# patrickltobing/shallow-wavenet

Measured on AMD Instinct MI355X. Metric: decoded samples/sec (22.05 kHz Laplacian AR decode, whole job), higher is better.
Workload: dtype f32

## Files before the change

shallow_wavenet_amd/csrc/swn_decode_bl6w.hip:

```cpp
#include <type_traits>
#include "swn_decode_bl6_common.hpp"
#include "swn_decode_internal.hpp"

#ifndef SWN_RES_SLICE
#define SWN_RES_SLICE 0
#endif
#ifndef SWN_ROTATE
#define SWN_ROTATE 1
#endif
#ifndef SWN_HANDOFF
#define SWN_HANDOFF 0
#endif
#ifndef SWN_OLDER2_MERGED
#define SWN_OLDER2_MERGED 1
#endif
#ifndef SWN_EARLY_ROWS
#define SWN_EARLY_ROWS 1
#endif

namespace {

using namespace swn_bl6;

constexpr int NG = 256;
constexpr int S = 128;
constexpr int O1 = 128;

template <int LPC_, bool EXT_>
struct Tw {
    static constexpr int LPC = LPC_;
    static constexpr bool EXT = EXT_;
    using Ext = Tw<LPC_, true>;
    static constexpr bool NEWFORM = !EXT_ && LPC_ == 0;
    static constexpr int NO = 2 + LPC_;
    static constexpr int WN = cmax(1, LPC_) + 1;
    static constexpr int ring_len(int l) { return pow2ceil((1 << l) + 1); }
    static constexpr int ring_off(int l) { int o = 0; for (int i = 0; i < l; ++i) o += ring_len(i) * H; return o; }
    static constexpr int PF = L * 2 * H;
    static constexpr int NZC = 64, NZB = 4;
    static constexpr int o_ring = 0;
    static constexpr int o_hcat = o_ring + ring_off(L);
    static constexpr int o_gp = o_hcat + L * H;
    static constexpr int o_bx = o_gp + 2 * PF;
    static constexpr int o_bd = o_bx + L * 2 * H;
    static constexpr int o_old = o_bd + L * 2 * H;
    static constexpr int o_wup = o_old + 2 * L * 2 * H;
    static constexpr int o_skip = o_wup + 256;
    static constexpr int o_p2 = o_skip + S;
    static constexpr int o_tnz = o_p2 + 4 * NO;
    static constexpr int o_cz = o_tnz + r4(NZB * NZC);
    static constexpr int o_w2 = o_cz + 5 * H;
    static constexpr int o_bias = o_w2 + NO * S + r4(NO);
    static constexpr int o_w1 = o_bias + S + O1;
    static constexpr int o_wl = o_w1 + 8 * O1 * 16;
    static constexpr int o_h0w = o_wl + 8 * NG * 4;
    static constexpr int o_ho = o_h0w + 3 * H;
    static constexpr int HO = 4, NHO = 128;
    static constexpr int o_end = o_ho + (NEWFORM && (SWN_HANDOFF & 1) && SWN_ROTATE ? NHO * HO : 0);
    static constexpr size_t lds_bytes = (size_t)o_end * sizeof(float);
    static constexpr int sess_old = ring_off(L);
    static constexpr int sess_win = sess_old + 2 * L * 2 * H;
    static constexpr int sess_floats = sess_win + r4(WN);
};

__device__ __forceinline__ float sum_quads(float v) {
    v += dpp_f<0x124>(v);
    v += dpp_f<0x128>(v);
    float w = v;
    asm("s_nop 1\n\tv_permlane16_swap_b32 %0, %1" : "+v"(v), "+v"(w));
    v += w;
    w = v;
    asm("s_nop 1\n\tv_permlane32_swap_b32 %0, %1" : "+v"(v), "+v"(w));
    return v + w;
}
__device__ __forceinline__ float quad_sum_by_parity(float own, float other) {
    float s = own + dpp_f<0xB1>(other);
    s += dpp_f<0x4E>(s);
    return s;
}
struct NoWork { __device__ __forceinline__ void operator()() const {} };
template <class T, int LAYER, int NQ = 2, class BEHIND = NoWork>
__device__ __forceinline__ void layer_a(float* lds, const float (&w)[2][16], const int q, const float wj, const int pb, const int po,
                                        const int ta, const float* xr, BEHIND&& behind = NoWork{}) {
    constexpr bool ROT = !std::is_same<typename std::decay<BEHIND>::type, NoWork>::value;
    const int o = ta >> 2, p = ta & 3, pr = p & 1;
    const float e_old = lds[T::o_old + po + LAYER * 2 * H + pr * H + o];
    const float g_gp = lds[T::o_gp + pb + LAYER * 2 * H + pr * H + o], g_bx = lds[T::o_bx + LAYER * 2 * H + pr * H + o];
    const float e_hp = xr[o];
    static_assert(NQ >= 0 && NQ <= 4, "early quads");
    float4 xq[4];
    if constexpr (ROT) {
#pragma unroll
        for (int m = 0; m < NQ; ++m) xq[m] = *reinterpret_cast<const float4*>(xr + 16 * p + 4 * m);
        __builtin_amdgcn_sched_barrier(0);
        behind();
        __builtin_amdgcn_sched_barrier(0);
    }
    const float e_gx = fmaf(wj, g_gp, g_bx);
    float az = 0.f, ac = 0.f;
#pragma unroll
    for (int m = 0; m < 4; ++m) {
        float4 x;
        if (ROT && m < NQ) x = xq[m];
        else x = *reinterpret_cast<const float4*>(xr + 16 * p + 4 * m);
        az = fmaf(w[0][4 * m], x.x, az); ac = fmaf(w[1][4 * m], x.x, ac);
        az = fmaf(w[0][4 * m + 1], x.y, az); ac = fmaf(w[1][4 * m + 1], x.y, ac);
        az = fmaf(w[0][4 * m + 2], x.z, az); ac = fmaf(w[1][4 * m + 2], x.z, ac);
        az = fmaf(w[0][4 * m + 3], x.w, az); ac = fmaf(w[1][4 * m + 3], x.w, ac);
    }
    const float sq = quad_sum_by_parity(pr ? ac : az, pr ? az : ac);
    __builtin_amdgcn_sched_barrier(0);
    if (p < 2) {
        const float sa = sq + e_old;
        const float v = e_gx * sa;
        const float e = exp_c(p == 0 ? -v : -2.f * fminf(fabsf(v), 64.f));
        const float r = rcp_c(1.f + e);
        const float res = p == 0 ? r : copysignf((1.f - e) * r, v);
        const float c = dpp_f<0xF5>(res);
        if (p == 0) {
            const float hn = (1.f - res) * c + res * e_hp;
            if (LAYER + 1 < L) {
                constexpr int R2 = T::ring_len(LAYER + 1 < L ? LAYER + 1 : LAYER);
                lds[T::o_ring + T::ring_off(LAYER + 1 < L ? LAYER + 1 : LAYER) + (q & (R2 - 1)) * H + o] = hn;
            }
            lds[T::o_hcat + LAYER * H + o] = hn;
        }
    }
    __builtin_amdgcn_sched_barrier(0);
}

template <class T, int LAYER, int MB = 4>
__device__ __forceinline__ void older_sum(const float* lds, const float (&w)[2][16], const int qn, const int tb, float& az, float& ac) {
    constexpr int dil = 1 << LAYER;
    constexpr int R = T::ring_len(LAYER);
    const int p = tb & 3;
    const float* ring = lds + T::o_ring + T::ring_off(LAYER);
    az = 0.f; ac = 0.f;
#pragma unroll
    for (int m = 0; m < 4; ++m) {
        const float4 x = *reinterpret_cast<const float4*>(ring + ((qn - dil) & (R - 1)) * H + 16 * p + 4 * m);
        float4 w0, w1;
        if (LAYER < L - 1) {
            w0 = make_float4(w[0][4 * m], w[0][4 * m + 1], w[0][4 * m + 2], w[0][4 * m + 3]);
            w1 = make_float4(w[1][4 * m], w[1][4 * m + 1], w[1][4 * m + 2], w[1][4 * m + 3]);
        } else {
            w0 = *reinterpret_cast<const float4*>(lds + T::o_wl + (m * NG + tb) * 4);
            w1 = *reinterpret_cast<const float4*>(lds + T::o_wl + ((4 + m) * NG + tb) * 4);
        }
        az = fmaf(w0.x, x.x, az); ac = fmaf(w1.x, x.x, ac);
        az = fmaf(w0.y, x.y, az); ac = fmaf(w1.y, x.y, ac);
        az = fmaf(w0.z, x.z, az); ac = fmaf(w1.z, x.z, ac);
        az = fmaf(w0.w, x.w, az); ac = fmaf(w1.w, x.w, ac);
        if (MB < 4 && m % MB == MB - 1) __builtin_amdgcn_sched_barrier(0);
    }
    az = sum4(az); ac = sum4(ac);
}
template <class T, int LAYER>
__device__ __forceinline__ void older_store(float* lds, const int qn, const int tb, const float az, const float ac) {
    const int o = tb >> 2, p = tb & 3, pr = p & 1;
    lds[T::o_old + (qn & 1) * (L * 2 * H) + LAYER * 2 * H + pr * H + o] = (p == 0 ? az : ac) + lds[T::o_bd + LAYER * 2 * H + pr * H + o];
}
template <class T, int LAYER, int MB = 4>
__device__ __forceinline__ void older_b(float* lds, const float (&w)[2][16], const int qn, const int tb) {
    float az, ac;
    older_sum<T, LAYER, MB>(lds, w, qn, tb, az, ac);
    if ((tb & 3) < 2) older_store<T, LAYER>(lds, qn, tb, az, ac);
}
template <class T>
__device__ __forceinline__ void older_last_rows(const float* lds, const int qn, const int tb, float4 (&x)[2], float4 (&w)[2][2]) {
    constexpr int LAYER = L - 1, dil = 1 << LAYER, R = T::ring_len(LAYER);
    const float* row = lds + T::o_ring + T::ring_off(LAYER) + ((qn - dil) & (R - 1)) * H + 16 * (tb & 3);
#pragma unroll
    for (int m = 0; m < 2; ++m) {
        x[m] = *reinterpret_cast<const float4*>(row + 4 * m);
        w[m][0] = *reinterpret_cast<const float4*>(lds + T::o_wl + (m * NG + tb) * 4);
        w[m][1] = *reinterpret_cast<const float4*>(lds + T::o_wl + ((4 + m) * NG + tb) * 4);
    }
}
template <class T>
__device__ __forceinline__ void older_last_x(float* lds, const float4 (&xe)[2], const float4 (&we)[2][2], const int qn, const int tb) {
    constexpr int LAYER = L - 1, dil = 1 << LAYER, R = T::ring_len(LAYER);
    const float* row = lds + T::o_ring + T::ring_off(LAYER) + ((qn - dil) & (R - 1)) * H + 16 * (tb & 3);
    float az = 0.f, ac = 0.f;
#pragma unroll
    for (int m = 0; m < 4; ++m) {
        float4 x, w0, w1;
        if (m < 2) { x = xe[m]; w0 = we[m][0]; w1 = we[m][1]; }
        else {
            x = *reinterpret_cast<const float4*>(row + 4 * m);
            w0 = *reinterpret_cast<const float4*>(lds + T::o_wl + (m * NG + tb) * 4);
            w1 = *reinterpret_cast<const float4*>(lds + T::o_wl + ((4 + m) * NG + tb) * 4);
        }
        az = fmaf(w0.x, x.x, az); ac = fmaf(w1.x, x.x, ac);
        az = fmaf(w0.y, x.y, az); ac = fmaf(w1.y, x.y, ac);
        az = fmaf(w0.z, x.z, az); ac = fmaf(w1.z, x.z, ac);
        az = fmaf(w0.w, x.w, az); ac = fmaf(w1.w, x.w, ac);
        if (m == 1) __builtin_amdgcn_sched_barrier(0);
    }
    az = sum4(az); ac = sum4(ac);
    if ((tb & 3) < 2) older_store<T, LAYER>(lds, qn, tb, az, ac);
}
template <int... LS> struct Layers {};
template <class T, int NW, int... LS>
__device__ __forceinline__ void older_bn(Layers<LS...>, float* lds, const float (&w)[NW][2][16], const int qn, const int tb) {
    static_assert(((LS < NW) && ...), "register-resident halves only");
    float az[sizeof...(LS)], ac[sizeof...(LS)];
    int k = 0;
    ((older_sum<T, LS>(lds, w[LS], qn, tb, az[k], ac[k]), ++k), ...);
    if ((tb & 3) < 2) {
        k = 0;
        ((older_store<T, LS>(lds, qn, tb, az[k], ac[k]), ++k), ...);
    }
}

template <class T, int LAYER>
__device__ __forceinline__ void older_rows(const float* lds, const int qn, const int tb, float4 (&x)[4]) {
    constexpr int dil = 1 << LAYER;
    constexpr int R = T::ring_len(LAYER);
    const float* row = lds + T::o_ring + T::ring_off(LAYER) + ((qn - dil) & (R - 1)) * H + 16 * (tb & 3);
#pragma unroll
    for (int m = 0; m < 4; ++m) x[m] = *reinterpret_cast<const float4*>(row + 4 * m);
}
__device__ __forceinline__ void older_sum_x(const float (&w)[2][16], const float4 (&x)[4], float& az, float& ac) {
    az = 0.f; ac = 0.f;
#pragma unroll
    for (int m = 0; m < 4; ++m) {
        az = fmaf(w[0][4 * m], x[m].x, az); ac = fmaf(w[1][4 * m], x[m].x, ac);
        az = fmaf(w[0][4 * m + 1], x[m].y, az); ac = fmaf(w[1][4 * m + 1], x[m].y, ac);
        az = fmaf(w[0][4 * m + 2], x[m].z, az); ac = fmaf(w[1][4 * m + 2], x[m].z, ac);
        az = fmaf(w[0][4 * m + 3], x[m].w, az); ac = fmaf(w[1][4 * m + 3], x[m].w, ac);
    }
    az = sum4(az); ac = sum4(ac);
}
template <class T, int... LS>
__device__ __forceinline__ void older_rows_n(Layers<LS...>, const float* lds, const int qn, const int tb, float4 (&x)[sizeof...(LS)][4]) {
    int k = 0;
    ((older_rows<T, LS>(lds, qn, tb, x[k]), ++k), ...);
}
template <class T, int NW, int... LS>
__device__ __forceinline__ void older_bn_x(Layers<LS...>, float* lds, const float (&w)[NW][2][16], const float4 (&x)[sizeof...(LS)][4],
                                           const int qn, const int tb) {
    static_assert(((LS < NW) && ...), "register-resident halves only");
    float az[sizeof...(LS)], ac[sizeof...(LS)];
    int k = 0;
    ((older_sum_x(w[LS], x[k], az[k], ac[k]), ++k), ...);
    if ((tb & 3) < 2) {
        k = 0;
        ((older_store<T, LS>(lds, qn, tb, az[k], ac[k]), ++k), ...);
    }
}

template <int LAYER>
__device__ __forceinline__ void skip_issue_b(__amdgpu_buffer_rsrc_t wsk2, float4 (&wsl)[8], const int tb, const unsigned step0) {
    const int r = tb >> 2, hp = tb & 3;
#pragma unroll
    for (int ps = 0; ps < 2; ++ps)
#pragma unroll
        for (int mm = 0; mm < 4; ++mm)
            wsl[ps * 4 + mm] = buf_ld4(wsk2, (unsigned)((r + 64 * ps) * 4 + hp) * 16u, (unsigned)((LAYER * 4 + mm) * S) * 64u + step0);
}
template <class T, int LAYER, bool REQ = true>
__device__ __forceinline__ void skip_roll_b(const float* lds, __amdgpu_buffer_rsrc_t wsk2, const float4 (&wcur)[8], float4 (&wnext)[8],
                                            float (&sacc)[2], const int tb, const unsigned step0) {
    static_assert(LAYER >= 1 && LAYER < L, "slice LAYER - 1 in flight, slice LAYER to request");
    const int r = tb >> 2, hp = tb & 3;
    float4 xs[4];
#pragma unroll
    for (int mm = 0; mm < 4; ++mm) xs[mm] = *reinterpret_cast<const float4*>(lds + T::o_hcat + (LAYER - 1) * H + 16 * mm + 4 * hp);
#pragma unroll
    for (int mm = 0; mm < 4; ++mm) {
#pragma unroll
        for (int ps = 0; ps < 2; ++ps) {
            const float4 x = xs[mm], w = wcur[ps * 4 + mm];
            sacc[ps] = fmaf(w.x, x.x, sacc[ps]); sacc[ps] = fmaf(w.y, x.y, sacc[ps]);
            sacc[ps] = fmaf(w.z, x.z, sacc[ps]); sacc[ps] = fmaf(w.w, x.w, sacc[ps]);
        }
        __builtin_amdgcn_sched_barrier(0);
#pragma unroll
        for (int ps = 0; ps < 2; ++ps)
            if (REQ) wnext[ps * 4 + mm] = buf_ld4(wsk2, (unsigned)((r + 64 * ps) * 4 + hp) * 16u, (unsigned)((LAYER * 4 + mm) * S) * 64u + step0);
        __builtin_amdgcn_sched_barrier(0);
    }
    asm volatile("" : "+v"(sacc[0]), "+v"(sacc[1]));
}
template <class T>
__device__ __forceinline__ void skip_last_b(float* lds, const float4 (&wsl)[8], const float (&sacc)[2], const int tb) {
    const int r = tb >> 2, hp = tb & 3;
    float part[2][4];
#pragma unroll
    for (int mm = 0; mm < 4; ++mm) {
        const float4 x = *reinterpret_cast<const float4*>(lds + T::o_hcat + (L - 1) * H + 16 * mm + 4 * hp);
#pragma unroll
        for (int ps = 0; ps < 2; ++ps) {
            const float4 w = wsl[ps * 4 + mm];
            part[ps][mm] = fmaf(w.w, x.w, fmaf(w.z, x.z, fmaf(w.y, x.y, w.x * x.x)));
        }
    }
    float s[2];
#pragma unroll
    for (int ps = 0; ps < 2; ++ps) s[ps] = sacc[ps] + ((part[ps][0] + part[ps][1]) + (part[ps][2] + part[ps][3]));
    const float t0 = s[0] + dpp_f<0xB1>(s[0]), t1 = s[1] + dpp_f<0xB1>(s[1]);
    const float v = (hp < 2 ? t0 : t1) + dpp_f<0x4E>(hp < 2 ? t1 : t0);
    if ((hp & 1) == 0) lds[T::o_skip + r + 32 * hp] = fmaxf(v, 0.f);
}

template <bool MOVE2> using OlderMergedT = typename std::conditional<MOVE2, Layers<2, 3, 4>, Layers<3, 4>>::type;
template <bool MOVE2> using OlderOut1T = typename std::conditional<MOVE2, Layers<0, 1>, Layers<0, 1, 2>>::type;
template <int E> struct Out1Split;
template <> struct Out1Split<2> { using Early = Layers<0, 1>; using Late = Layers<>; };
template <> struct Out1Split<1> { using Early = Layers<0>; using Late = Layers<1>; };
template <> struct Out1Split<0> { using Early = Layers<>; using Late = Layers<0, 1>; };

template <class T, bool GA, bool STREAM, bool POOL = false>
__device__ __forceinline__ void decode_body(const Bl6Args& a, float* lds) {
    constexpr bool EXT = T::EXT;
    static_assert(!STREAM || EXT, "streamed chunks run the extended mode");
    constexpr bool grpA = GA;
    const int tid = threadIdx.x, b = POOL ? 0 : blockIdx.x;
    __builtin_assume(GA ? tid < NG : tid >= NG);
    const int tg = tid & (NG - 1);
    const float* __restrict__ P = a.P;
    const int U = a.U;
    const int s0 = STREAM ? a.step0 : 0;
    const bool resume = STREAM && a.resume;
    const int fb0 = STREAM ? s0 / U : 0;

    for (int e = tid; e < T::o_end; e += NT) lds[e] = 0.f;
    __syncthreads();
    for (int e = tid; e < L * 2 * H; e += NT) {
        lds[T::o_bx + e] = P[a.y.bx + e];
        const float bd = P[a.y.bd + e];
        lds[T::o_bd + e] = bd;
        lds[T::o_old + e] = bd;
    }
    for (int e = tid; e < U; e += NT) lds[T::o_wup + e] = P[a.y.wup + e];
    for (int e = tid; e < H; e += NT) lds[T::o_cz + e] = P[a.y.cb + e];
    for (int e = tid; e < S; e += NT) lds[T::o_bias + e] = P[a.y.bsk + e];
    for (int e = tid; e < O1; e += NT) lds[T::o_bias + S + e] = P[a.y.b1 + e];
    for (int e = tid; e < 2 * H; e += NT) { lds[T::o_cz + H + e] = P[a.y.cv + e]; lds[T::o_cz + 3 * H + e] = P[a.y.cc + e]; }
    for (int e = tid; e < T::NO * S; e += NT) lds[T::o_w2 + e] = P[a.y.w2 + (size_t)(e / S) * r4(S) + (e % S)];
    for (int e = tid; e < T::NO; e += NT) lds[T::o_w2 + T::NO * S + e] = P[a.y.b2 + e];
    for (int e = tid; e < 8 * O1 * 16; e += NT) lds[T::o_w1 + e] = P[a.y.w12 + e];
    const __amdgpu_buffer_rsrc_t condr =
        make_rsrc(a.cond + (size_t)b * a.Tf * a.N, (unsigned)((size_t)a.Tf * a.N * sizeof(float)));
    auto load_frame = [&](int fr) {
        float* dst = lds + T::o_gp + (fr & 1) * T::PF;
#pragma unroll
        for (int it = 0; it < (T::PF / 4 + NT - 1) / NT; ++it) {
            const int e4 = it * NT + tid;
            if (e4 < T::PF / 4)
                *reinterpret_cast<float4*>(dst + 4 * e4) =
                    buf_ld4(condr, (unsigned)tid * 16u, (unsigned)(fr * a.N * 4 + it * NT * 16));
        }
    };
    for (int fr = fb0; fr < fb0 + 2 && fr < a.Tf; ++fr) load_frame(fr);
    constexpr int NWR = grpA ? L : L - 1;
    float wreg[NWR][2][16];
    {
        const int o = tg >> 2, p = tg & 3, k = grpA ? 1 : 0;
#pragma unroll
        for (int l = 0; l < L; ++l)
#pragma unroll
            for (int r = 0; r < 2; ++r) {
                const float4* src = reinterpret_cast<const float4*>(P + a.y.wd + (((size_t)l * 2 * H + o + r * H) * 2 + k) * H + 16 * p);
#pragma unroll
                for (int v = 0; v < 4; ++v) {
                    const float4 t = src[v];
                    if (l == L - 1 && !grpA) {
                        *reinterpret_cast<float4*>(lds + T::o_wl + ((r * 4 + v) * NG + tg) * 4) = t;
                    } else {
                        float (&wr)[16] = wreg[l < NWR ? l : 0][r];
                        wr[4 * v] = t.x; wr[4 * v + 1] = t.y; wr[4 * v + 2] = t.z; wr[4 * v + 3] = t.w;
                    }
                }
            }
    }
    __syncthreads();
    const float* sess_b = STREAM ? a.sess + (size_t)b * T::sess_floats : nullptr;
    int tcp = tid;
    asm volatile("" : "+v"(tcp));
    if (resume) {
        for (int e = tcp; e < T::ring_off(L); e += NT) lds[T::o_ring + e] = sess_b[e];
        for (int e = tcp; e < 2 * L * 2 * H; e += NT) lds[T::o_old + e] = sess_b[T::sess_old + e];
        __syncthreads();
    }

    int fb = fb0, tb0 = fb0 * U;
    const int n_pro = RF;
    auto cond_taps = [&](int q, float& wj, int& pb) {
        const int t0 = q - RF;
        const int tlo = t0 < 0 ? 0 : t0;
        if (tlo >= tb0 + U) {
            fb += 1; tb0 += U;
            if (fb + 1 < a.Tf) load_frame(fb + 1);
        }
        int rel = tlo - tb0;
        int fsel = fb;
        if (rel >= U) { rel -= U; fsel = fb + 1; }
        rel = rel < U ? rel : U - 1;
        wj = lds[T::o_wup + rel];
        pb = (fsel & 1) * T::PF;
    };

    auto input_seed = [&](int q) {
        if (tid < H) {
            const int o = tid;
            float acc = c_b;
#pragma unroll
            for (int k = 0; k < 2; ++k) {
                const int r = q - (1 - k);
                if (r >= 0) acc += fmaf(k ? c_v1 : c_v0, 0.f, k ? c_c1 : c_c0);
            }
            lds[T::o_ring + (q & 1) * H + o] = ssign(acc);
        }
    };
    float win[T::WN];
#pragma unroll
    for (int k = 0; k < T::WN; ++k) win[k] = 0.f;
    if (EXT && a.seed) win[T::WN - 1] = reinterpret_cast<const float*>(a.seed)[b];
    if (resume) {
#pragma unroll
        for (int k = 0; k < T::WN; ++k) win[k] = sess_b[T::sess_win + k];
    }
    const int wv = __builtin_amdgcn_readfirstlane(tg >> 6);
    float kcb = 0.f, kv0 = 0.f, kv1 = 0.f, kc0 = 0.f, kc1 = 0.f;
    if (grpA) { const int o = tg & (H - 1); kcb = c_b; kv0 = c_v0; kv1 = c_v1; kc0 = c_c0; kc1 = c_c1; }
    auto h0_row = [&](int qn) -> int {
        return wv == 0 ? T::o_ring + (qn & 1) * H : T::o_h0w + (wv - 1) * H;
    };
    auto input_gen = [&](int row) {
        if constexpr (grpA) {
            float acc = kcb;
            acc += fmaf(kv0, win[T::WN - 2], kc0);
            acc += fmaf(kv1, win[T::WN - 1], kc1);
            lds[row + (tg & (H - 1))] = ssign(acc);
            lds_fence_compiler();
        }
    };
#ifdef SWN_DIAG_NOSIDE
    constexpr bool NOSIDE = T::NEWFORM;
#else
    constexpr bool NOSIDE = false;
#endif
#ifdef SWN_DIAG_NOSTREAM
    constexpr bool NOSTREAM = T::NEWFORM;
#else
    constexpr bool NOSTREAM = false;
#endif
    constexpr bool HOFF = T::NEWFORM && (SWN_HANDOFF & 7) && SWN_ROTATE;
    constexpr bool HO_ST = HOFF && (SWN_HANDOFF & 1), HO_RF = HOFF && (SWN_HANDOFF & 2), HO_NZ = HOFF && (SWN_HANDOFF & 4);
    constexpr bool MOVE2 = T::NEWFORM && SWN_OLDER2_MERGED;
    using OlderMerged = OlderMergedT<MOVE2>;
    using OlderOut1 = OlderOut1T<MOVE2>;
    constexpr int NOUT1 = MOVE2 ? 2 : 3;
    constexpr int NEARLY = MOVE2 ? SWN_EARLY_ROWS : NOUT1;
    static_assert(NEARLY >= 0 && NEARLY <= NOUT1, "early rows");
    constexpr bool NZG = HO_NZ ? !grpA : grpA;
    const int tn = HO_NZ ? tg : tid;
    float e_next = 0.f;
    auto noise_load = [&](int c) {
        const int step = c * T::NZC + tn - 64;
        if (step < a.n_steps) e_next = a.noise[(size_t)b * a.n_steps + step];
    };
    auto noise_chunk = [&](int c) {
        if (NZG && tn >= 64 && tn < 128) {
            const int k = tn - 64, step = c * T::NZC + k;
            if (step < a.n_steps) {
                const float e = EXT ? swn_noise_laplace_at(a.nz, b, step, s0 + step, 0, a.n_steps, 1) : e_next;
                const float sg = (e > 0.f) ? 1.f : ((e < 0.f) ? -1.f : 0.f);
                lds[T::o_tnz + (c & (T::NZB - 1)) * T::NZC + k] = sg * log1pf(-2.f * fabsf(e));
            }
            if (!EXT) noise_load(c + 1);
        }
    };
    if (!EXT && NZG && tn >= 64 && tn < 128) noise_load(0);
    noise_chunk(0);
    noise_chunk(1);

    const __amdgpu_buffer_rsrc_t wsk2 = make_rsrc(P + a.y.wsk2, (unsigned)(L * S * 64 * sizeof(float)));
    constexpr bool NEWFORM = T::NEWFORM;
    constexpr int RES = (grpA || !NEWFORM) ? -1 : SWN_RES_SLICE;
    static_assert(RES == -1 || RES == 0 || RES == L - 1, "the first or the last slice");
    float4 wres[8];
    if constexpr (RES == 0) skip_issue_b<0>(wsk2, wres, tg, 0u);
    if constexpr (RES == L - 1) skip_issue_b<L - 1>(wsk2, wres, tg, 0u);

#ifdef SWN_STAMP
    unsigned long long tw[9] = {0, 0, 0, 0, 0, 0, 0, 0, 0}, tv[6] = {0, 0, 0, 0, 0, 0}, tstep = 0, tlast = 0, tbeg = 0;
#define SWN_BAR(k) { tw[k] += __builtin_amdgcn_s_memtime() - tlast; lds_barrier(); tlast = __builtin_amdgcn_s_memtime(); }
#define SWN_WAIT_STAMP(k) { asm volatile("" :: "v"(wsl[0].x)); tv[k] += __builtin_amdgcn_s_memtime() - tlast; }
#define SWN_PRE(k) { tw[k] += __builtin_amdgcn_s_memtime() - tlast; asm volatile("s_waitcnt lgkmcnt(0)" ::: "memory"); }
#define SWN_BAR_KEEP(k, N) { lds_barrier_keep<N>(); tlast = __builtin_amdgcn_s_memtime(); }
#else
#define SWN_BAR(k) lds_barrier();
#define SWN_WAIT_STAMP(k)
#define SWN_PRE(k)
#define SWN_BAR_KEEP(k, N) lds_barrier_keep<N>();
#endif
#define SWN_PHASE_WORK(LAYER, GEN, X0)                                                                                \
    if constexpr (grpA) layer_a<T, LAYER>(lds, wreg[LAYER], q, wj, pb, po, tg,                                         \
                                          LAYER == 0 ? (X0) : lds + T::o_ring + T::ring_off(LAYER) +                   \
                                                                  (q & (T::ring_len(LAYER) - 1)) * H);                 \
    else {                                                                                                             \
        if (GEN) {    \
                      \
                      \
                      \
            if (LAYER == 0) { if (RES != 0) skip_issue_b<0>(wsk2, wsl, tg, step0); }                                   \
            else if (LAYER == 1 && RES == 0) skip_roll_b<T, 1, !NOSTREAM>(lds, wsk2, wres, wsl, sacc, tg, step0);      \
            else { SWN_WAIT_STAMP(LAYER > 0 ? LAYER - 1 : 0)                                                           \
                   skip_roll_b<T, (LAYER > 0 ? LAYER : 1), !(LAYER == L - 1 && RES == L - 1) && !NOSTREAM>(lds, wsk2, wsl, wsl, sacc, tg, step0); } \
            __builtin_amdgcn_sched_barrier(0);                                                                         \
        }                                                                                                              \
        if (!(GEN)) older_b<T, LAYER>(lds, wreg[LAYER < NWR ? LAYER : 0], q + 1, tg);                                  \
        else if (LAYER == 0) older_bn<T>(OlderMerged{}, lds, wreg, q + 1, tg);                                         \
        __builtin_amdgcn_sched_barrier(0);                                                                             \
    }
#define SWN_PHASE(LAYER, GEN, X0) SWN_PHASE_WORK(LAYER, GEN, X0) if (GEN) { SWN_BAR(LAYER) } else lds_barrier();

#pragma unroll 1
    for (int q = resume ? n_pro : 0; q < n_pro; ++q) {
        float wj; int pb;
        float4 wsl[8]; float sacc[2]; const unsigned step0 = 0;
        cond_taps(q, wj, pb);
        const int po = (q & 1) * (L * 2 * H);
        input_seed(q);
        lds_barrier();
        const float* x0 = lds + T::o_ring + (q & 1) * H;
        SWN_PHASE(0, false, x0) SWN_PHASE(1, false, x0) SWN_PHASE(2, false, x0) SWN_PHASE(3, false, x0)
        SWN_PHASE(4, false, x0) SWN_PHASE(5, false, x0)
        (void)wsl; (void)sacc; (void)step0;
    }

    int rel_c = s0 - fb0 * U;
    bool fill_c = false;
    float wj_c = 0.f;
    int pb_c = 0, po_c = 0, x0_c = 0;
    auto taps_ahead = [&](int qn) {
        wj_c = lds[T::o_wup + rel_c];
        pb_c = (fb & 1) * T::PF;
        po_c = (qn & 1) * (L * 2 * H);
        x0_c = h0_row(qn);
        asm volatile("" : "+s"(pb_c), "+s"(po_c), "+s"(x0_c));
    };
    auto frame_advance = [&]() {
        rel_c += 1;
        const bool cross = rel_c >= U;
        if (cross) { rel_c = 0; fb += 1; }
        fill_c = cross && fb + 1 < a.Tf;
    };
    if constexpr (grpA) taps_ahead(RF + s0);
    input_gen(x0_c);
#ifdef SWN_STAMP
    tlast = tbeg = __builtin_amdgcn_s_memtime();
#endif
    constexpr bool ROT = SWN_ROTATE && NEWFORM;
    constexpr int ROTQ = 2;
    float sv_p = 0.f, acc_p = 0.f;
    const __amdgpu_buffer_rsrc_t outr =
        make_rsrc(reinterpret_cast<float*>(a.out) + (size_t)b * a.n_steps, (unsigned)((size_t)a.n_steps * sizeof(float)));
    const __amdgpu_buffer_rsrc_t headr =
        make_rsrc(HEADS_ON && a.heads ? a.heads + (size_t)b * a.n_steps * T::NO : nullptr,
                  HEADS_ON && a.heads ? (unsigned)((size_t)a.n_steps * T::NO * sizeof(float)) : 0u);
    auto store_step = [&](const int ip) __attribute__((always_inline)) {
        if constexpr (grpA && ROT) {
            if (tid == 0) __builtin_amdgcn_raw_buffer_store_b32(__builtin_bit_cast(unsigned, sv_p), outr, 0u, (unsigned)ip * 4u, 0);
            if (wv == 0 && (tg & 63) < T::NO)
                __builtin_amdgcn_raw_buffer_store_b32(__builtin_bit_cast(unsigned, acc_p), headr, (unsigned)(tg & 63) * 4u,
                                                      (unsigned)(ip * T::NO) * 4u, 0);
        } else if constexpr (grpA) {
            if (tid == 0) reinterpret_cast<float*>(a.out)[(size_t)b * a.n_steps + (size_t)ip] = sv_p;
            if (HEADS_ON && a.heads && wv == 0 && (tg & 63) < T::NO) a.heads[((size_t)b * a.n_steps + ip) * T::NO + (tg & 63)] = acc_p;
        }
    };
    static_assert(!HOFF || (T::PF / 4 <= NG && T::NO == 2 && T::HO == 4), "one refill request per thread, a slot is {head, head, sample, -}");
    auto ho_write = [&](const int ip) __attribute__((always_inline)) {
        if constexpr (grpA) {
            if (wv == 0) {
                float* const slot = lds + T::o_ho + (ip & (T::NHO - 1)) * T::HO;
                slot[(tg & 63) < T::NO ? (tg & 63) : T::NO - 1] = acc_p;
                slot[T::NO] = sv_p;
            }
        }
    };
    auto load_frame_b = [&](int fr) {
        if (tg < T::PF / 4)
            *reinterpret_cast<float4*>(lds + T::o_gp + (fr & 1) * T::PF + 4 * tg) =
                buf_ld4(condr, (unsigned)tg * 16u, (unsigned)(fr * a.N * 4));
    };
    auto store_chunk_b = [&](const int c) __attribute__((always_inline)) {
        const int step = c * 64 + tg;
        if (tg < 64 && step < a.n_steps) {
            const float4 v = *reinterpret_cast<const float4*>(lds + T::o_ho + (step & (T::NHO - 1)) * T::HO);
            __builtin_amdgcn_raw_buffer_store_b32(__builtin_bit_cast(unsigned, v.z), outr, (unsigned)tg * 4u, (unsigned)c * 256u, 0);
            using u2 = unsigned __attribute__((ext_vector_type(2)));
            u2 h; h.x = __builtin_bit_cast(unsigned, v.x); h.y = __builtin_bit_cast(unsigned, v.y);
            __builtin_amdgcn_raw_buffer_store_b64(h, headr, (unsigned)tg * 8u, (unsigned)c * 512u, 0);
        }
    };
    auto gen_step = [&](const int i) __attribute__((always_inline)) {
        const int q = RF + s0 + i;
        const float wj = wj_c;
        const int pb = pb_c, po = po_c;
        if constexpr (grpA && !ROT) {
            if (fill_c) load_frame(fb + 1);
        }
        auto behind0 = [&]() __attribute__((always_inline)) {
            if constexpr (NOSIDE) return;
            if constexpr (!HO_NZ) { if ((i & (T::NZC - 1)) == 0) noise_chunk((i >> 6) + 2); }
            if constexpr (!HO_RF) { if (fill_c) load_frame(fb + 1); }
            if constexpr (HO_ST) { if (i > 0) ho_write(i - 1); }
            else { if (i > 0) store_step(i - 1); }
        };
        float4 wsl[8];
        float sacc[2] = {0.f, 0.f};
        if constexpr (!grpA) {
            const float bs0 = lds[T::o_bias + (tg >> 2)], bs1 = lds[T::o_bias + (tg >> 2) + 64];
            if ((tg & 3) == 0) { sacc[0] = bs0; sacc[1] = bs1; }
        }
        unsigned step0 = 0;
        asm volatile("" : "+s"(step0));
        const float* x0 = lds + x0_c;
#ifdef SWN_DIAG_NOSIDE_B
        constexpr bool SIDE_B = false;
#else
        constexpr bool SIDE_B = HOFF && !grpA && !NOSIDE;
#endif
        if constexpr (SIDE_B) {
            __builtin_amdgcn_sched_barrier(0);
            if constexpr (HO_NZ) { if ((i & (T::NZC - 1)) == 0) noise_chunk((i >> 6) + 2); }
            if constexpr (HO_RF) { if (fill_c) load_frame_b(fb + 1); }
            if constexpr (HO_ST) { if ((i & 63) == 1 && i > 1) store_chunk_b((i >> 6) - 1); }
            __builtin_amdgcn_sched_barrier(0);
        }
        if constexpr (NOSTREAM && !grpA) {
#pragma unroll
            for (int k = 0; k < 8; ++k) asm volatile("" : "=v"(wsl[k].x), "=v"(wsl[k].y), "=v"(wsl[k].z), "=v"(wsl[k].w));
        }
        if constexpr (grpA && ROT) {
            layer_a<T, 0, ROTQ>(lds, wreg[0], q, wj, pb, po, tg, x0, behind0);
            SWN_BAR(0)
        } else {
            SWN_PHASE(0, true, x0)
        }
        SWN_PHASE(1, true, x0) SWN_PHASE(2, true, x0) SWN_PHASE(3, true, x0)
        SWN_PHASE(4, true, x0)
        constexpr bool EARLY5 = T::LPC == 0;
        float4 xl[2], wl[2][2];
        SWN_PHASE_WORK(5, true, x0)
        if constexpr (grpA && EARLY5) {
            SWN_PRE(5)
            lds_fence_compiler();
            __builtin_amdgcn_sched_barrier(0);
            older_last_rows<T>(lds, q + 1, tg + (int)step0, xl, wl);
            __builtin_amdgcn_sched_barrier(0);
            SWN_BAR_KEEP(5, 6)
        } else {
            SWN_BAR(5)
        }
        constexpr bool ROLL1 = T::LPC == 0;
        using Split = Out1Split<MOVE2 ? NEARLY : 2>;
        float4 xo[cmax(NEARLY, 1)][4];
        float4 w1e[2][2];
        if constexpr (!grpA) {
            if constexpr (RES == L - 1) skip_last_b<T>(lds, wres, sacc, tg);
            else { SWN_WAIT_STAMP(5) skip_last_b<T>(lds, wsl, sacc, tg); }
            SWN_PRE(6)
            lds_fence_compiler();
            __builtin_amdgcn_sched_barrier(0);
            if constexpr (!MOVE2) {
                older_rows_n<T>(OlderOut1{}, lds, q + 1, tg, xo);
                __builtin_amdgcn_sched_barrier(0);
                SWN_BAR_KEEP(6, 12)
            } else if constexpr (NEARLY > 0) {
                older_rows_n<T>(typename Split::Early{}, lds, q + 1, tg, xo);
                __builtin_amdgcn_sched_barrier(0);
                SWN_BAR_KEEP(6, 4 * NEARLY)
            } else {
                SWN_BAR_KEEP(6, 0)
            }
        } else {
            if constexpr (EARLY5) older_last_x<T>(lds, xl, wl, q + 1, tg + (int)step0);
            else older_b<T, L - 1, 2>(lds, wreg[L - 1], q + 1, tg + (int)step0);
            if constexpr (ROLL1) {
                SWN_PRE(6)
                lds_fence_compiler();
                __builtin_amdgcn_sched_barrier(0);
#pragma unroll
                for (int mm = 0; mm < 2; ++mm)
#pragma unroll
                    for (int r = 0; r < 2; ++r)
                        w1e[mm][r] = *reinterpret_cast<const float4*>(lds + T::o_w1 + ((mm * O1 + (tg >> 2) + 64 * r) * 4 + (tg & 3)) * 4);
                __builtin_amdgcn_sched_barrier(0);
                SWN_BAR_KEEP(6, 4)
            } else {
                SWN_BAR(6)
            }
        }
        if constexpr (grpA) {
            const int hr = tg >> 2, hp = tg & 3;
            float a0 = 0.f, a1 = 0.f, b0 = 0.f, b1 = 0.f;
            auto X = [&](int mm) { return *reinterpret_cast<const float4*>(lds + T::o_skip + 16 * mm + 4 * hp); };
            auto W = [&](int mm, int r) { return *reinterpret_cast<const float4*>(lds + T::o_w1 + ((mm * O1 + hr + 64 * r) * 4 + hp) * 4); };
            auto fma8 = [&](int mm, const float4& x0, const float4& w0, const float4& w1) {
                float& acc = (mm & 1) ? a1 : a0;
                float& bcc = (mm & 1) ? b1 : b0;
                acc = fmaf(w0.x, x0.x, acc); acc = fmaf(w0.y, x0.y, acc); acc = fmaf(w0.z, x0.z, acc); acc = fmaf(w0.w, x0.w, acc);
                bcc = fmaf(w1.x, x0.x, bcc); bcc = fmaf(w1.y, x0.y, bcc); bcc = fmaf(w1.z, x0.z, bcc); bcc = fmaf(w1.w, x0.w, bcc);
            };
            float e_b1[2] = {0.f, 0.f}, e_w2[2] = {0.f, 0.f}, e_b2 = 0.f;
            const int e_kc = hp < T::NO ? hp : T::NO - 1;
            if constexpr (ROLL1) {
                static_assert(T::NO <= 4, "one round of out_2 rows");
                float4 xr[3] = {X(0), X(1), X(2)};
                __builtin_amdgcn_sched_barrier(0);
#pragma unroll
                for (int mm = 0; mm < 8; ++mm) {
                    fma8(mm, xr[mm % 3], w1e[mm % 2][0], w1e[mm % 2][1]);
                    __builtin_amdgcn_sched_barrier(0);
                    if (mm + 2 < 8) { w1e[mm % 2][0] = W(mm + 2, 0); w1e[mm % 2][1] = W(mm + 2, 1); }
                    if (mm + 3 < 8) xr[mm % 3] = X(mm + 3);
                    if (mm == 5) {
                        e_b1[0] = lds[T::o_bias + S + hr]; e_b1[1] = lds[T::o_bias + S + hr + 64];
                        e_w2[0] = lds[T::o_w2 + e_kc * S + hr]; e_w2[1] = lds[T::o_w2 + e_kc * S + hr + 64];
                    }
                    if (mm == 6) e_b2 = lds[T::o_w2 + T::NO * S + e_kc];
                    __builtin_amdgcn_sched_barrier(0);
                }
            } else {
#pragma unroll
                for (int mm = 0; mm < 8; ++mm) {
                    fma8(mm, X(mm), W(mm, 0), W(mm, 1));
                    if ((mm & 3) == 3) __builtin_amdgcn_sched_barrier(0);
                }
            }
            const float v = sum4(a0 + a1), u = sum4(b0 + b1);
            if constexpr (ROLL1) {
                const float o1a = fmaxf(v + e_b1[0], 0.f), o1b = fmaxf(u + e_b1[1], 0.f);
                const float pz = sum_quads(fmaf(e_w2[1], o1b, fmaf(e_w2[0], o1a, tg < 4 ? e_b2 : 0.f)));
                if ((tg & 63) < 4 && hp < T::NO) lds[T::o_p2 + 4 * hp + wv] = pz;
            } else {
                const float o1a = fmaxf(v + lds[T::o_bias + S + hr], 0.f), o1b = fmaxf(u + lds[T::o_bias + S + hr + 64], 0.f);
#pragma unroll
                for (int j = 0; j < (T::NO + 3) / 4; ++j) {
                    const int k = hp + 4 * j, kc = k < T::NO ? k : T::NO - 1;
                    const float* w2 = lds + T::o_w2 + kc * S;
                    const float b2 = lds[T::o_w2 + T::NO * S + kc];
                    const float pz = sum_quads(fmaf(w2[hr + 64], o1b, fmaf(w2[hr], o1a, tg < 4 ? b2 : 0.f)));
                    if ((tg & 63) < 4 && k < T::NO) lds[T::o_p2 + 4 * k + wv] = pz;
                }
            }
        } else if constexpr (!MOVE2) {
            older_bn_x<T>(OlderOut1{}, lds, wreg, xo, q + 1, tg);
        } else {
            if constexpr (NEARLY > 0) older_bn_x<T>(typename Split::Early{}, lds, wreg, xo, q + 1, tg);
            if constexpr (NEARLY < NOUT1) older_bn<T>(typename Split::Late{}, lds, wreg, q + 1, tg);
        }
        SWN_BAR(7)
        if constexpr (grpA) {
            const int ln = tg & 63;
            float tz = 0.f;
            if constexpr (!EXT) tz = lds[T::o_tnz + (i & (T::NZB * T::NZC - 1))];
            float fv = 0.f;
            if (a.forced) fv = reinterpret_cast<const float*>(a.forced)[(size_t)b * a.n_steps + i];
            const float4 pz = *reinterpret_cast<const float4*>(lds + T::o_p2 + 4 * (ln < T::NO ? ln : T::NO - 1));
            __builtin_amdgcn_sched_barrier(0);
            frame_advance();
            taps_ahead(q + 1);
            __builtin_amdgcn_sched_barrier(0);
            const float acc = (pz.x + pz.y) + (pz.z + pz.w);
            float o2[T::NO];
#pragma unroll
            for (int k = 0; k < T::NO; ++k) o2[k] = __builtin_bit_cast(float, __builtin_amdgcn_readlane(__builtin_bit_cast(int, acc), k));
            float sv;
            {
#pragma clang fp contract(off)
                const float mu = o2[0];
                const float bsc = sigm(o2[1]);
                float lpv = 0.f;
#pragma unroll
                for (int k = 0; k < T::LPC; ++k) lpv += o2[2 + T::LPC - 1 - k] * win[T::WN - T::LPC + k];
                const float t = bsc * (EXT ? lds[T::o_tnz + ((i >> 6) & (T::NZB - 1)) * T::NZC + (i & (T::NZC - 1))] : tz);
                sv = (T::LPC > 0) ? (lpv + mu) - t : mu - t;
                sv = fminf(fmaxf(sv, -1.f), 1.f);
                float fd = a.forced ? fv : sv;
                asm volatile("" : "+v"(fd));
#pragma unroll
                for (int k = 0; k + 1 < T::WN; ++k) win[k] = win[k + 1];
                win[T::WN - 1] = fd;
            }
            if (i + 1 < a.n_steps) input_gen(x0_c);
            __builtin_amdgcn_sched_barrier(0);
            if constexpr (ROT) { sv_p = sv; acc_p = acc; }
            else {
                if (tid == 0) reinterpret_cast<float*>(a.out)[(size_t)b * a.n_steps + (size_t)i] = sv;
                if (HEADS_ON && a.heads && wv == 0 && ln < T::NO) a.heads[((size_t)b * a.n_steps + i) * T::NO + ln] = acc;
            }
        }
        if constexpr (HO_RF && !grpA) frame_advance();
#ifdef SWN_STAMP
        if constexpr (grpA) tw[8] += __builtin_amdgcn_s_memtime() - tlast;
#endif
    };
    if constexpr (ROT) {
#pragma unroll 1
        for (int i = 0; i < a.n_steps; ++i) gen_step(i);
        if constexpr (HO_ST) {
            if constexpr (grpA) { if (a.n_steps > 0) ho_write(a.n_steps - 1); }
            lds_barrier();
            if constexpr (!grpA) {
                for (int c = a.n_steps >= 66 ? ((a.n_steps - 66) >> 6) + 1 : 0; c * 64 < a.n_steps; ++c) store_chunk_b(c);
            }
        } else if (a.n_steps > 0) store_step(a.n_steps - 1);
    } else {
#pragma unroll 1
        for (int i0 = 0; i0 < a.n_steps; i0 += T::NZC) {
            noise_chunk((i0 >> 6) + 2);
            const int iend = i0 + T::NZC < a.n_steps ? i0 + T::NZC : a.n_steps;
#pragma unroll 1
            for (int i = i0; i < iend; ++i) gen_step(i);
        }
    }
#ifdef SWN_STAMP
    { const unsigned long long tn = __builtin_amdgcn_s_memtime(); tw[0] += tn - tlast; tstep = tn - tbeg; }
#endif
    if constexpr (STREAM) {
        __syncthreads();
        float* so = a.sess + (size_t)b * T::sess_floats;
        tcp = tid;
        asm volatile("" : "+v"(tcp));
        for (int e = tcp; e < T::ring_off(L); e += NT) so[e] = lds[T::o_ring + e];
        for (int e = tcp; e < 2 * L * 2 * H; e += NT) so[T::sess_old + e] = lds[T::o_old + e];
        if (tid == 0) {
#pragma unroll
            for (int k = 0; k < T::WN; ++k) so[T::sess_win + k] = win[k];
        }
    }
#undef SWN_PHASE
#undef SWN_PHASE_WORK
#undef SWN_BAR
#undef SWN_WAIT_STAMP
#undef SWN_PRE
#undef SWN_BAR_KEEP
#ifdef SWN_STAMP
    if ((tid == 0 || tid == 64 || tid == NG) && b == 0 && a.heads) {
        float* h = a.heads + (tid == 0 ? 0 : tid == 64 ? 30 : 10);
        for (int k = 0; k < 9; ++k) h[k] = (float)((double)tw[k] / (double)a.n_steps);
        if (tid == 0) h[9] = (float)((double)tstep / (double)a.n_steps);
        else if (tid == NG) for (int k = 0; k < 6; ++k) h[10 + k] = (float)((double)tv[k] / (double)a.n_steps);
    }
#endif
}

template <class T, bool STREAM = false>
__global__ __launch_bounds__(NT) void decode_bl6w_kernel(const Bl6Args a) {
    extern __shared__ __attribute__((aligned(16))) float lds[];
    if (threadIdx.x < NG) decode_body<T, true, STREAM>(a, lds);
    else decode_body<T, false, STREAM>(a, lds);
}

template <class T, bool MODELS = false>
__global__ __launch_bounds__(NT) void decode_bl6w_pool_kernel(
    const typename std::conditional<MODELS, Bl6PoolModelsArgs, Bl6PoolArgs>::type p) {
    extern __shared__ __attribute__((aligned(16))) float lds[];
    static_assert(T::EXT, "pools run the extended mode");
    Bl6Args a = p.c;
    if constexpr (MODELS) a.P = swn_pool_model(p.m);
    if (!swn_pool_entry_args(a, p.t, 1, 1, T::NO)) return;
    a.sess += (size_t)swn_pool_slot(p.t) * T::sess_floats;
    if (threadIdx.x < NG) decode_body<T, true, true, true>(a, lds);
    else decode_body<T, false, true, true>(a, lds);
}

template <class T>
__global__ __launch_bounds__(NT) void decode_bl6w_pool_wide_kernel(const Bl6PoolWideArgs p) {
    extern __shared__ __attribute__((aligned(16))) float lds[];
    static_assert(T::EXT, "pools run the extended mode");
    Bl6Args a = p.c;
    const SwnPoolWideRow row = swn_pool_wide_row(p.rows);
    a.P = row.model;
    if (!swn_pool_entry_args(a, row.e, 1, 1, T::NO)) return;
    a.sess += (size_t)row.e.slot * T::sess_floats;
    if (threadIdx.x < NG) decode_body<T, true, true, true>(a, lds);
    else decode_body<T, false, true, true>(a, lds);
}

bool bl6w_applies(const SwnGeom& g) {
    return g.bl6 && g.U <= 256 && g.U >= 2 && !g.audio_in && g.kind == SWN_KIND_LAPLACE && g.S == 128 && g.O1 == 128 &&
           g.seg == 1 && (g.lpc == 0 || g.lpc == 4);
}

template <class F>
int with_tw(const SwnGeom& g, F&& f) {
    if (!bl6w_applies(g)) return SWN_E_UNSUPPORTED;
    if (g.lpc == 0) return f(Tw<0, false>{});
    return f(Tw<4, false>{});
}

}

int swn_decode_bl6w_run(const SwnDecodeCall& c) {
    const hipStream_t st = c.hip_stream;
    if (c.wide) {
        Bl6PoolWideArgs p;
        fill_args(p.c, c);
        p.rows = c.wide;
        return with_tw(c.g, [&](auto tw) {
            using T = typename decltype(tw)::Ext;
            return launch_kernel(decode_bl6w_pool_wide_kernel<T>, T::lds_bytes, c.batch, p, st, "swn_decode_pool_chunk_wide(bl6w)");
        });
    }
    if (c.pool) {
        Bl6PoolModelsArgs p;
        fill_args(p.c, c);
        p.t = *c.pool;
        if (c.models) p.m = *c.models;
        return with_tw(c.g, [&](auto tw) {
            using T = typename decltype(tw)::Ext;
            if (c.models)
                return launch_kernel(decode_bl6w_pool_kernel<T, true>, T::lds_bytes, c.batch, p, st, "swn_decode_pool_chunk_models(bl6w)");
            const Bl6PoolArgs& p1 = p;
            return launch_kernel(decode_bl6w_pool_kernel<T>, T::lds_bytes, c.batch, p1, st, "swn_decode_pool_chunk(bl6w)");
        });
    }
    Bl6Args a;
    fill_args(a, c);
    return with_tw(c.g, [&](auto t) {
        using T = decltype(t);
        using X = typename T::Ext;
        static_assert(T::lds_bytes <= 160 * 1024 && X::lds_bytes <= 160 * 1024, "LDS budget");
        if (c.stream) return launch_kernel(decode_bl6w_kernel<X, true>, X::lds_bytes, a.B, a, st, "swn_decode(bl6w)");
        if (wants_ext(a)) return launch_kernel(decode_bl6w_kernel<X>, X::lds_bytes, a.B, a, st, "swn_decode(bl6w)");
        return launch_kernel(decode_bl6w_kernel<T>, T::lds_bytes, a.B, a, st, "swn_decode(bl6w)");
    });
}

size_t swn_decode_bl6w_session_floats(const SwnGeom& g) {
    int n = 0;
    with_tw(g, [&](auto t) { n = decltype(t)::sess_floats; return SWN_OK; });
    return (size_t)n;
}
```

Baseline: 407,000.

## Lead skip-weight slice loads ahead and read skip inputs from ring rows

Reworks the skip-weight streaming in the generator warps so that part of each next slice's buffer loads is issued at the head of the current roll, and the same number of loads is deferred from its tail. The aim is to keep more global loads in flight across layer barriers. It also makes the skip path read each layer's hidden row from the dilation ring, which lets non-final layers skip the separate hcat store. Diagnostic-only exp and timer variants are added behind macros. The cost is more schedule complexity and added register pressure, and the slice ordering must stay correct for the rolled wcur/wnext aliasing.

```diff
diff --git a/shallow_wavenet_amd/csrc/swn_decode_bl6w.hip b/shallow_wavenet_amd/csrc/swn_decode_bl6w.hip
--- a/shallow_wavenet_amd/csrc/swn_decode_bl6w.hip
+++ b/shallow_wavenet_amd/csrc/swn_decode_bl6w.hip
@@ -16,6 +16,19 @@
 #endif
 #ifndef SWN_EARLY_ROWS
 #define SWN_EARLY_ROWS 1
+#endif
+#ifndef SWN_LEAD
+#define SWN_LEAD 1
+#endif
+#ifndef SWN_RINGX
+#define SWN_RINGX 1
+#endif
+#ifdef SWN_STAMP
+#define SWN_TDEF_PARAM , unsigned long long& tdef
+#define SWN_TDEF_ARG(k) , td[k]
+#else
+#define SWN_TDEF_PARAM
+#define SWN_TDEF_ARG(k)
 #endif
 
 namespace {
@@ -32,6 +45,8 @@
     static constexpr bool EXT = EXT_;
     using Ext = Tw<LPC_, true>;
     static constexpr bool NEWFORM = !EXT_ && LPC_ == 0;
+    static constexpr int LEAD = NEWFORM ? SWN_LEAD : 0;
+    static constexpr bool RINGX = NEWFORM && SWN_RINGX;
     static constexpr int NO = 2 + LPC_;
     static constexpr int WN = cmax(1, LPC_) + 1;
     static constexpr int ring_len(int l) { return pow2ceil((1 << l) + 1); }
@@ -113,8 +128,13 @@
     if (p < 2) {
         const float sa = sq + e_old;
         const float v = e_gx * sa;
+#ifdef SWN_DIAG_PLAINEXP
+        const float e = __builtin_amdgcn_exp2f((p == 0 ? -v : -2.f * fminf(fabsf(v), 64.f)) * 1.44269504f);
+        const float r = __builtin_amdgcn_rcpf(1.f + e);
+#else
         const float e = exp_c(p == 0 ? -v : -2.f * fminf(fabsf(v), 64.f));
         const float r = rcp_c(1.f + e);
+#endif
         const float res = p == 0 ? r : copysignf((1.f - e) * r, v);
         const float c = dpp_f<0xF5>(res);
         if (p == 0) {
@@ -123,7 +143,7 @@
                 constexpr int R2 = T::ring_len(LAYER + 1 < L ? LAYER + 1 : LAYER);
                 lds[T::o_ring + T::ring_off(LAYER + 1 < L ? LAYER + 1 : LAYER) + (q & (R2 - 1)) * H + o] = hn;
             }
-            lds[T::o_hcat + LAYER * H + o] = hn;
+            if (!T::RINGX || LAYER + 1 >= L) lds[T::o_hcat + LAYER * H + o] = hn;
         }
     }
     __builtin_amdgcn_sched_barrier(0);
@@ -259,16 +279,40 @@
         for (int mm = 0; mm < 4; ++mm)
             wsl[ps * 4 + mm] = buf_ld4(wsk2, (unsigned)((r + 64 * ps) * 4 + hp) * 16u, (unsigned)((LAYER * 4 + mm) * S) * 64u + step0);
 }
-template <class T, int LAYER, bool REQ = true>
-__device__ __forceinline__ void skip_roll_b(const float* lds, __amdgpu_buffer_rsrc_t wsk2, const float4 (&wcur)[8], float4 (&wnext)[8],
-                                            float (&sacc)[2], const int tb, const unsigned step0) {
+template <class T, int LAYER, bool REQ = true, int HEAD = 0, int DEFER = 0, bool HEAD_OWN = false>
+__device__ __forceinline__ void skip_roll_b(const float* lds, __amdgpu_buffer_rsrc_t wsk2, float4 (&wcur)[8], float4 (&wnext)[8],
+                                            float (&sacc)[2], const int tb, const unsigned step0, const int q SWN_TDEF_PARAM) {
     static_assert(LAYER >= 1 && LAYER < L, "slice LAYER - 1 in flight, slice LAYER to request");
+    static_assert(HEAD >= 0 && HEAD <= 4 && DEFER >= 0 && DEFER <= 4, "at most half a slice leads");
     const int r = tb >> 2, hp = tb & 3;
+    auto request = [&](float4 (&dst)[8], const int slice, const int k) __attribute__((always_inline)) {
+        const int mm = k >> 1, ps = k & 1;
+        dst[ps * 4 + mm] = buf_ld4(wsk2, (unsigned)((r + 64 * ps) * 4 + hp) * 16u, (unsigned)((slice * 4 + mm) * S) * 64u + step0);
+    };
+    constexpr int R = T::ring_len(LAYER);
+    const float* xrow = T::RINGX ? lds + T::o_ring + T::ring_off(LAYER) + (q & (R - 1)) * H : lds + T::o_hcat + (LAYER - 1) * H;
     float4 xs[4];
 #pragma unroll
-    for (int mm = 0; mm < 4; ++mm) xs[mm] = *reinterpret_cast<const float4*>(lds + T::o_hcat + (LAYER - 1) * H + 16 * mm + 4 * hp);
+    for (int mm = 0; mm < 4; ++mm) xs[mm] = *reinterpret_cast<const float4*>(xrow + 16 * mm + 4 * hp);
+    if constexpr (REQ && HEAD > 0) {
+        __builtin_amdgcn_sched_barrier(0);
+#pragma unroll
+        for (int k = 0; k < HEAD; ++k) {
+            if (HEAD_OWN) request(wnext, LAYER, k);
+            else request(wcur, LAYER - 1, 8 - HEAD + k);
+        }
+        __builtin_amdgcn_sched_barrier(0);
+    }
 #pragma unroll
     for (int mm = 0; mm < 4; ++mm) {
+#ifdef SWN_STAMP
+        if (!HEAD_OWN && HEAD > 0 && mm == (8 - HEAD) >> 1) {
+            const unsigned long long t0 = __builtin_amdgcn_s_memtime();
+            asm volatile("s_waitcnt lgkmcnt(0)" ::: "memory");
+            asm volatile("" :: "v"(wcur[((8 - HEAD) & 1) * 4 + mm].x));
+            tdef += __builtin_amdgcn_s_memtime() - t0;
+        }
+#endif
 #pragma unroll
         for (int ps = 0; ps < 2; ++ps) {
             const float4 x = xs[mm], w = wcur[ps * 4 + mm];
@@ -277,8 +321,10 @@
         }
         __builtin_amdgcn_sched_barrier(0);
 #pragma unroll
-        for (int ps = 0; ps < 2; ++ps)
-            if (REQ) wnext[ps * 4 + mm] = buf_ld4(wsk2, (unsigned)((r + 64 * ps) * 4 + hp) * 16u, (unsigned)((LAYER * 4 + mm) * S) * 64u + step0);
+        for (int ps = 0; ps < 2; ++ps) {
+            const int k = 2 * mm + ps;
+            if (REQ && k >= (HEAD_OWN ? HEAD : 0) && k < 8 - DEFER) request(wnext, LAYER, k);
+        }
         __builtin_amdgcn_sched_barrier(0);
     }
     asm volatile("" : "+v"(sacc[0]), "+v"(sacc[1]));
@@ -481,12 +527,14 @@
     constexpr bool NEWFORM = T::NEWFORM;
     constexpr int RES = (grpA || !NEWFORM) ? -1 : SWN_RES_SLICE;
     static_assert(RES == -1 || RES == 0 || RES == L - 1, "the first or the last slice");
+    constexpr int LEADB = RES == 0 ? T::LEAD : 0;
+    static_assert(LEADB == 0 || LEADB == 1 || LEADB == 2 || LEADB == 4, "one load, a quarter or a half of a slice");
     float4 wres[8];
     if constexpr (RES == 0) skip_issue_b<0>(wsk2, wres, tg, 0u);
     if constexpr (RES == L - 1) skip_issue_b<L - 1>(wsk2, wres, tg, 0u);
 
 #ifdef SWN_STAMP
-    unsigned long long tw[9] = {0, 0, 0, 0, 0, 0, 0, 0, 0}, tv[6] = {0, 0, 0, 0, 0, 0}, tstep = 0, tlast = 0, tbeg = 0;
+    unsigned long long tw[9] = {0, 0, 0, 0, 0, 0, 0, 0, 0}, tv[6] = {0, 0, 0, 0, 0, 0}, td[5] = {0, 0, 0, 0, 0}, tstep = 0, tlast = 0, tbeg = 0;
 #define SWN_BAR(k) { tw[k] += __builtin_amdgcn_s_memtime() - tlast; lds_barrier(); tlast = __builtin_amdgcn_s_memtime(); }
 #define SWN_WAIT_STAMP(k) { asm volatile("" :: "v"(wsl[0].x)); tv[k] += __builtin_amdgcn_s_memtime() - tlast; }
 #define SWN_PRE(k) { tw[k] += __builtin_amdgcn_s_memtime() - tlast; asm volatile("s_waitcnt lgkmcnt(0)" ::: "memory"); }
@@ -507,9 +555,13 @@
                       \
                       \
             if (LAYER == 0) { if (RES != 0) skip_issue_b<0>(wsk2, wsl, tg, step0); }                                   \
-            else if (LAYER == 1 && RES == 0) skip_roll_b<T, 1, !NOSTREAM>(lds, wsk2, wres, wsl, sacc, tg, step0);      \
+                      \
+            else if (LAYER == 1 && RES == 0)                                                                           \
+                skip_roll_b<T, 1, !NOSTREAM, LEADB, LEADB, true>(lds, wsk2, wres, wsl, sacc, tg, step0, q SWN_TDEF_ARG(0)); \
             else { SWN_WAIT_STAMP(LAYER > 0 ? LAYER - 1 : 0)                                                           \
-                   skip_roll_b<T, (LAYER > 0 ? LAYER : 1), !(LAYER == L - 1 && RES == L - 1) && !NOSTREAM>(lds, wsk2, wsl, wsl, sacc, tg, step0); } \
+                   skip_roll_b<T, (LAYER > 0 ? LAYER : 1), !(LAYER == L - 1 && RES == L - 1) && !NOSTREAM,             \
+                               (LAYER >= 2 ? LEADB : 0), (LAYER < L - 1 ? LEADB : 0)>(lds, wsk2, wsl, wsl, sacc, tg, step0, q \
+                                                                                      SWN_TDEF_ARG(LAYER > 0 ? LAYER - 1 : 0)); } \
             __builtin_amdgcn_sched_barrier(0);                                                                         \
         }                                                                                                              \
         if (!(GEN)) older_b<T, LAYER>(lds, wreg[LAYER < NWR ? LAYER : 0], q + 1, tg);                                  \
@@ -847,7 +899,10 @@
         float* h = a.heads + (tid == 0 ? 0 : tid == 64 ? 30 : 10);
         for (int k = 0; k < 9; ++k) h[k] = (float)((double)tw[k] / (double)a.n_steps);
         if (tid == 0) h[9] = (float)((double)tstep / (double)a.n_steps);
-        else if (tid == NG) for (int k = 0; k < 6; ++k) h[10 + k] = (float)((double)tv[k] / (double)a.n_steps);
+        else if (tid == NG) {
+            for (int k = 0; k < 6; ++k) h[10 + k] = (float)((double)tv[k] / (double)a.n_steps);
+            for (int k = 0; k < 5; ++k) h[34 + k] = (float)((double)td[k] / (double)a.n_steps);
+        }
     }
 #endif
 }
```

Measured after the change: 411,800, median of 6. 1.01x the previous value.
